# lab-emi/CleanUMamba

Measured on AMD Instinct MI355X. Metric: audio samples/sec/node (train step, E8, 10s@16kHz), higher is better.
Workload: dtype f16; 1 GPU; CleanUMamba-E8 (41.4M) full train step: fwd + L1 + multi-res STFT loss + bwd + grad all-reduce + clip + Adam; 10 s @ 16 kHz clips; global_batch=16, batch_per_gpu=16, clip_samples=160000, parallelism=dp1, weights=random init (reference init, seed 0)

## Files before the change

cleanumamba_amd/csrc/pack.hip:

```cpp
#include "common.h"

namespace cum {

template <typename TD>
struct Vec4;
template <>
struct Vec4<float> {
  typedef float4 type;
  static __device__ __forceinline__ type make(float a, float b, float c, float d) { return make_float4(a, b, c, d); }
};
template <>
struct Vec4<__bf16> {
  typedef __attribute__((ext_vector_type(4))) __bf16 type;
  static __device__ __forceinline__ type make(float a, float b, float c, float d) {
    type v = {(__bf16)a, (__bf16)b, (__bf16)c, (__bf16)d};
    return v;
  }
};

template <>
struct Vec4<f16> {
  typedef __attribute__((ext_vector_type(4))) _Float16 type;
  static __device__ __forceinline__ type make(float a, float b, float c, float d) {
    type v = {(f16)a, (f16)b, (f16)c, (f16)d};
    return v;
  }
};

template <typename TS, typename TD>
__global__ __launch_bounds__(256) void gather_kernel(const TS *__restrict__ src, const int32_t *__restrict__ idx,
                                                     TD *__restrict__ dst, int64_t n) {
  typedef typename Vec4<TD>::type V;
  const int64_t stride = (int64_t)gridDim.x * 256 * 8;
  for (int64_t i0 = ((int64_t)blockIdx.x * 256 + threadIdx.x) * 8; i0 < n; i0 += stride) {
    if (i0 + 7 < n) {
      const int4 j = *reinterpret_cast<const int4 *>(idx + i0), k = *reinterpret_cast<const int4 *>(idx + i0 + 4);
      const float v0 = j.x < 0 ? 0.f : (float)src[j.x], v1 = j.y < 0 ? 0.f : (float)src[j.y];
      const float v2 = j.z < 0 ? 0.f : (float)src[j.z], v3 = j.w < 0 ? 0.f : (float)src[j.w];
      const float v4 = k.x < 0 ? 0.f : (float)src[k.x], v5 = k.y < 0 ? 0.f : (float)src[k.y];
      const float v6 = k.z < 0 ? 0.f : (float)src[k.z], v7 = k.w < 0 ? 0.f : (float)src[k.w];
      *reinterpret_cast<V *>(dst + i0) = Vec4<TD>::make(v0, v1, v2, v3);
      *reinterpret_cast<V *>(dst + i0 + 4) = Vec4<TD>::make(v4, v5, v6, v7);
    } else {
      for (int64_t i = i0; i < n; ++i) {
        const int32_t jj = idx[i];
        dst[i] = (TD)(jj < 0 ? 0.f : (float)src[jj]);
      }
    }
  }
}

constexpr int PACK_PAD = -2147483647 - 1;
struct PackJob {
  int64_t dst_off;
  int32_t rows, cols;
  int32_t row_tab, col_tab;
  int32_t transpose;
  int32_t runs8;
};

template <typename TD>
__global__ __launch_bounds__(256) void pack2d_kernel(const float *__restrict__ src, const PackJob *__restrict__ jobs,
                                                    const int32_t *__restrict__ tiles, const int32_t *__restrict__ tables,
                                                    TD *__restrict__ dst) {
  typedef typename Vec4<TD>::type V;
  __shared__ __attribute__((aligned(16))) TD tile[64][72];
  const int tid = threadIdx.x;
  const PackJob j = jobs[tiles[3 * blockIdx.x]];
  const int r0 = tiles[3 * blockIdx.x + 1] * 64, c0 = tiles[3 * blockIdx.x + 2] * 64;
  const int32_t *rt = tables + j.row_tab, *ct = tables + j.col_tab;
  TD *out = dst + j.dst_off;
  if (j.transpose) {
    const int r = r0 + (tid & 63), cw = c0 + 16 * (tid >> 6);
    const int ro = r < j.rows ? rt[r] : PACK_PAD;
#pragma unroll
    for (int cc = 0; cc < 16; ++cc) {
      const int c = cw + cc;
      const int co = c < j.cols ? ct[c] : PACK_PAD;
      const float v = (ro == PACK_PAD || co == PACK_PAD) ? 0.f : src[(int64_t)ro + co];
      tile[tid & 63][16 * (tid >> 6) + cc] = (TD)v;
    }
    __syncthreads();
  }
  const int cg = 8 * (tid & 7);
#pragma unroll
  for (int h = 0; h < 2; ++h) {
    const int rl = (tid >> 3) + 32 * h, r = r0 + rl, c = c0 + cg;
    if (r >= j.rows || c >= j.cols) continue;
    if (j.transpose) {
      *reinterpret_cast<uint4 *>(out + (int64_t)r * j.cols + c) = *reinterpret_cast<const uint4 *>(&tile[rl][cg]);
      if constexpr (sizeof(TD) == 4)
        *reinterpret_cast<uint4 *>(out + (int64_t)r * j.cols + c + 4) = *reinterpret_cast<const uint4 *>(&tile[rl][cg + 4]);
    } else {
      const int ro = rt[r];
      float v[8];
      if (j.runs8) {
        const int co = ct[c];
        const bool pad = ro == PACK_PAD || co == PACK_PAD;
        const float *q = src + (pad ? 0 : (int64_t)ro + co);
        if (j.runs8 == 2) {
          const float4 a = pad ? make_float4(0.f, 0.f, 0.f, 0.f) : *reinterpret_cast<const float4 *>(q);
          const float4 b = pad ? make_float4(0.f, 0.f, 0.f, 0.f) : *reinterpret_cast<const float4 *>(q + 4);
          v[0] = a.x; v[1] = a.y; v[2] = a.z; v[3] = a.w; v[4] = b.x; v[5] = b.y; v[6] = b.z; v[7] = b.w;
        } else {
#pragma unroll
          for (int i = 0; i < 8; ++i) v[i] = pad ? 0.f : q[i];
        }
      } else {
#pragma unroll
        for (int i = 0; i < 8; ++i) {
          const int co = ct[c + i];
          v[i] = (ro == PACK_PAD || co == PACK_PAD) ? 0.f : src[(int64_t)ro + co];
        }
      }
      *reinterpret_cast<V *>(out + (int64_t)r * j.cols + c) = Vec4<TD>::make(v[0], v[1], v[2], v[3]);
      *reinterpret_cast<V *>(out + (int64_t)r * j.cols + c + 4) = Vec4<TD>::make(v[4], v[5], v[6], v[7]);
    }
  }
}

}

using namespace cum;

extern "C" int cum_pack2d(const float *src, const void *jobs, const int32_t *tiles, int32_t n_tiles, const int32_t *tables,
                          int32_t dst_dtype, void *dst, void *stream) {
  CUM_REQUIRE(dtype_ok(dst_dtype), "pack2d: dst dtype must be CUM_F32 / CUM_BF16 / CUM_F16");
  CUM_REQUIRE(n_tiles >= 0, "pack2d: negative tile count");
  if (n_tiles == 0) return CUM_OK;
  CUM_REQUIRE(src && jobs && tiles && tables && dst && ((uintptr_t)dst & 15) == 0 && ((uintptr_t)src & 15) == 0,
              "pack2d: null or misaligned pointer");
  hipStream_t st = (hipStream_t)stream;
  const PackJob *pj = static_cast<const PackJob *>(jobs);
  if (dst_dtype == CUM_F16)
    hipLaunchKernelGGL(pack2d_kernel<f16>, dim3(n_tiles), dim3(256), 0, st, src, pj, tiles, tables, (f16 *)dst);
  else if (dst_dtype == CUM_BF16)
    hipLaunchKernelGGL(pack2d_kernel<__bf16>, dim3(n_tiles), dim3(256), 0, st, src, pj, tiles, tables, (__bf16 *)dst);
  else
    hipLaunchKernelGGL(pack2d_kernel<float>, dim3(n_tiles), dim3(256), 0, st, src, pj, tiles, tables, (float *)dst);
  CUM_CHECK_LAUNCH();
  return CUM_OK;
}

extern "C" int cum_gather(int32_t src_dtype, const void *src, const int32_t *idx, int64_t n, int32_t dst_dtype,
                          void *dst, void *stream) {
  CUM_REQUIRE(dtype_ok(src_dtype) && dtype_ok(dst_dtype) && !(is16(src_dtype) && is16(dst_dtype) && src_dtype != dst_dtype),
              "gather: dtypes must be CUM_F32 / CUM_BF16 / CUM_F16 (no bf16 <-> f16 conversion)");
  CUM_REQUIRE(n >= 0, "gather: negative length");
  if (n == 0) return CUM_OK;
  CUM_REQUIRE(src && idx && dst && ((uintptr_t)idx & 15) == 0 && ((uintptr_t)dst & 15) == 0,
              "gather: null or misaligned pointer");
  const int64_t want = (n + 2047) / 2048;
  dim3 grid((unsigned)(want < 8192 ? want : 8192)), block(256);
  hipStream_t st = (hipStream_t)stream;
  if (src_dtype == CUM_F32 && dst_dtype == CUM_F16)
    hipLaunchKernelGGL((gather_kernel<float, f16>), grid, block, 0, st, (const float *)src, idx, (f16 *)dst, n);
  else if (src_dtype == CUM_F16 && dst_dtype == CUM_F32)
    hipLaunchKernelGGL((gather_kernel<f16, float>), grid, block, 0, st, (const f16 *)src, idx, (float *)dst, n);
  else if (src_dtype == CUM_F16)
    hipLaunchKernelGGL((gather_kernel<f16, f16>), grid, block, 0, st, (const f16 *)src, idx, (f16 *)dst, n);
  else if (src_dtype == CUM_F32 && dst_dtype == CUM_F32)
    hipLaunchKernelGGL((gather_kernel<float, float>), grid, block, 0, st, (const float *)src, idx, (float *)dst, n);
  else if (src_dtype == CUM_F32)
    hipLaunchKernelGGL((gather_kernel<float, __bf16>), grid, block, 0, st, (const float *)src, idx, (__bf16 *)dst, n);
  else if (dst_dtype == CUM_F32)
    hipLaunchKernelGGL((gather_kernel<__bf16, float>), grid, block, 0, st, (const __bf16 *)src, idx, (float *)dst, n);
  else
    hipLaunchKernelGGL((gather_kernel<__bf16, __bf16>), grid, block, 0, st, (const __bf16 *)src, idx, (__bf16 *)dst, n);
  CUM_CHECK_LAUNCH();
  return CUM_OK;
}
```

Measured before the change: 128.1 million audio samples/s.

## Make pack2d persistent with software-pipelined tile loads and double-buffered LDS

The pack kernel now launches a capped persistent grid sized to CU count times a fixed occupancy factor, and each workgroup walks a contiguous range of tiles. Table lookups and global loads for the next tile are issued while the current tile is being stored. LDS is double-buffered, and the non-transposed gather path now also goes through LDS. Branchy pad handling is replaced by redirecting padded reads to a zero buffer, with readlane broadcast of column indices. The aim is to hide gather latency and cut launch and tail overhead, at the cost of more registers and complexity in what is likely a small slice of the train step.

```diff
diff --git a/cleanumamba_amd/csrc/pack.hip b/cleanumamba_amd/csrc/pack.hip
--- a/cleanumamba_amd/csrc/pack.hip
+++ b/cleanumamba_amd/csrc/pack.hip
@@ -59,64 +59,169 @@
   int32_t runs8;
 };
 
+constexpr int PACK_WG_PER_CU = 8;
+
+struct PackTile {
+  int32_t job, tr, tc;
+};
+
+struct PackTab {
+  int32_t e0, e1, e2;
+};
+
+__device__ __forceinline__ bool pack_direct(const PackJob &j) { return !j.transpose && j.runs8; }
+
+__device__ __forceinline__ PackTile pack_tile(const int32_t *__restrict__ tiles, int t) {
+  PackTile p;
+  p.job = tiles[3 * t], p.tr = tiles[3 * t + 1], p.tc = tiles[3 * t + 2];
+  return p;
+}
+
+__device__ __forceinline__ PackTab pack_tab(const int32_t *__restrict__ tables, const PackJob &j, const PackTile &p,
+                                            int tid) {
+  const int32_t *rt = tables + j.row_tab, *ct = tables + j.col_tab;
+  PackTab t;
+  t.e2 = 0;
+  if (pack_direct(j)) {
+    const int r = 64 * p.tr + (tid >> 3), c = 64 * p.tc + 8 * (tid & 7);
+    t.e0 = rt[min(r, j.rows - 1)];
+    t.e1 = rt[min(r + 32, j.rows - 1)];
+    t.e2 = ct[min(c, j.cols - 8)];
+  } else if (j.transpose) {
+    t.e0 = rt[min(64 * p.tr + (tid & 63), j.rows - 1)];
+    t.e1 = ct[min(64 * p.tc + 16 * (tid >> 6) + (tid & 15), j.cols - 1)];
+  } else {
+    t.e0 = ct[min(64 * p.tc + (tid & 63), j.cols - 1)];
+    t.e1 = rt[min(64 * p.tr + 16 * (tid >> 6) + (tid & 15), j.rows - 1)];
+  }
+  return t;
+}
+
+__device__ __attribute__((aligned(16))) float pack_zeros[8];
+typedef float PackF4 __attribute__((ext_vector_type(4)));
+typedef const __attribute__((address_space(1))) float *PackSrc;
+typedef const __attribute__((address_space(1))) PackF4 *PackSrc4;
+
+__device__ __forceinline__ uintptr_t pack_addr(const float *src, int ro, int co, bool inside) {
+  const bool live = inside & (ro != PACK_PAD) & (co != PACK_PAD);
+  return live ? (uintptr_t)src + 4 * (uintptr_t)((int64_t)ro + co) : (uintptr_t)pack_zeros;
+}
+
+__device__ __forceinline__ void pack_load(const float *__restrict__ src, const PackJob &j, const PackTile &p, const PackTab &t,
+                                          int tid, float (&x)[16]) {
+  if (pack_direct(j)) {
+    const int r = 64 * p.tr + (tid >> 3);
+    const bool cin = 64 * p.tc + 8 * (tid & 7) < j.cols;
+#pragma unroll
+    for (int h = 0; h < 2; ++h) {
+      const uintptr_t q = pack_addr(src, h ? t.e1 : t.e0, t.e2, cin & (r + 32 * h < j.rows));
+      if (j.runs8 == 2) {
+        const PackF4 a = *(PackSrc4)q, b = *(PackSrc4)(q + 16);
+        x[8 * h + 0] = a.x, x[8 * h + 1] = a.y, x[8 * h + 2] = a.z, x[8 * h + 3] = a.w;
+        x[8 * h + 4] = b.x, x[8 * h + 5] = b.y, x[8 * h + 6] = b.z, x[8 * h + 7] = b.w;
+      } else {
+#pragma unroll
+        for (int i = 0; i < 8; ++i) x[8 * h + i] = *(PackSrc)(q + 4 * i);
+      }
+    }
+  } else {
+    const int own_n = j.transpose ? j.rows : j.cols, other_n = j.transpose ? j.cols : j.rows;
+    const bool own_in = 64 * (j.transpose ? p.tr : p.tc) + (tid & 63) < own_n;
+    const int first = 64 * (j.transpose ? p.tc : p.tr) + 16 * (tid >> 6);
+#pragma unroll
+    for (int k = 0; k < 16; ++k) {
+      const int e = __builtin_amdgcn_readlane(t.e1, k);
+      x[k] = *(PackSrc)pack_addr(src, t.e0, e, own_in & (first + k < other_n));
+    }
+  }
+}
+
+template <typename TD>
+__device__ __forceinline__ void pack_store8(TD *p, const float *v) {
+  typedef typename Vec4<TD>::type V;
+  if constexpr (sizeof(TD) == 4) {
+    *reinterpret_cast<V *>(p) = Vec4<TD>::make(v[0], v[1], v[2], v[3]);
+    *reinterpret_cast<V *>(p + 4) = Vec4<TD>::make(v[4], v[5], v[6], v[7]);
+  } else {
+    typedef TD V8 __attribute__((ext_vector_type(8)));
+    const V8 o = {(TD)v[0], (TD)v[1], (TD)v[2], (TD)v[3], (TD)v[4], (TD)v[5], (TD)v[6], (TD)v[7]};
+    *reinterpret_cast<V8 *>(p) = o;
+  }
+}
+
 template <typename TD>
 __global__ __launch_bounds__(256) void pack2d_kernel(const float *__restrict__ src, const PackJob *__restrict__ jobs,
-                                                    const int32_t *__restrict__ tiles, const int32_t *__restrict__ tables,
-                                                    TD *__restrict__ dst) {
-  typedef typename Vec4<TD>::type V;
-  __shared__ __attribute__((aligned(16))) TD tile[64][72];
+                                                    const int32_t *__restrict__ tiles, int32_t n_tiles,
+                                                    const int32_t *__restrict__ tables, TD *__restrict__ dst) {
+  __shared__ __attribute__((aligned(16))) TD tile[2][64][72];
   const int tid = threadIdx.x;
-  const PackJob j = jobs[tiles[3 * blockIdx.x]];
-  const int r0 = tiles[3 * blockIdx.x + 1] * 64, c0 = tiles[3 * blockIdx.x + 2] * 64;
-  const int32_t *rt = tables + j.row_tab, *ct = tables + j.col_tab;
-  TD *out = dst + j.dst_off;
-  if (j.transpose) {
-    const int r = r0 + (tid & 63), cw = c0 + 16 * (tid >> 6);
-    const int ro = r < j.rows ? rt[r] : PACK_PAD;
-#pragma unroll
-    for (int cc = 0; cc < 16; ++cc) {
-      const int c = cw + cc;
-      const int co = c < j.cols ? ct[c] : PACK_PAD;
-      const float v = (ro == PACK_PAD || co == PACK_PAD) ? 0.f : src[(int64_t)ro + co];
-      tile[tid & 63][16 * (tid >> 6) + cc] = (TD)v;
-    }
-    __syncthreads();
-  }
-  const int cg = 8 * (tid & 7);
-#pragma unroll
-  for (int h = 0; h < 2; ++h) {
-    const int rl = (tid >> 3) + 32 * h, r = r0 + rl, c = c0 + cg;
-    if (r >= j.rows || c >= j.cols) continue;
-    if (j.transpose) {
-      *reinterpret_cast<uint4 *>(out + (int64_t)r * j.cols + c) = *reinterpret_cast<const uint4 *>(&tile[rl][cg]);
-      if constexpr (sizeof(TD) == 4)
-        *reinterpret_cast<uint4 *>(out + (int64_t)r * j.cols + c + 4) = *reinterpret_cast<const uint4 *>(&tile[rl][cg + 4]);
+  const int t0 = (int)((int64_t)blockIdx.x * n_tiles / gridDim.x), t1 = (int)((int64_t)(blockIdx.x + 1) * n_tiles / gridDim.x);
+  if (t0 >= t1) return;
+  const int last = t1 - 1;
+  PackTile p0 = pack_tile(tiles, t0), p1 = pack_tile(tiles, min(t0 + 1, last)), p2 = pack_tile(tiles, min(t0 + 2, last)),
+           p3 = pack_tile(tiles, min(t0 + 3, last));
+  PackJob j0 = jobs[p0.job], j1 = jobs[p1.job], j2 = jobs[p2.job];
+  float xa[16], xb[16];
+#pragma unroll
+  for (int i = 0; i < 16; ++i) xa[i] = xb[i] = 0.f;
+  pack_load(src, j0, p0, pack_tab(tables, j0, p0, tid), tid, xa);
+  PackTab b1 = pack_tab(tables, j1, p1, tid);
+  int buf = 0;
+  auto step = [&](int t, float (&x)[16], float (&nx)[16]) {
+    const PackTab b2 = pack_tab(tables, j2, p2, tid);
+    if (t < last) pack_load(src, j1, p1, b1, tid, nx);
+    const PackJob j3 = jobs[p3.job];
+    const PackTile p4 = pack_tile(tiles, min(t + 4, last));
+    TD *out = dst + j0.dst_off;
+    const int r0 = 64 * p0.tr, c = 64 * p0.tc + 8 * (tid & 7);
+    if (!pack_direct(j0)) {
+      TD(*tl)[72] = tile[buf];
+      if (j0.transpose) {
+        pack_store8(&tl[tid & 63][16 * (tid >> 6)], x);
+        pack_store8(&tl[tid & 63][16 * (tid >> 6) + 8], x + 8);
+      } else {
+#pragma unroll
+        for (int k = 0; k < 16; ++k) tl[16 * (tid >> 6) + k][tid & 63] = (TD)x[k];
+      }
+      __syncthreads();
+#pragma unroll
+      for (int h = 0; h < 2; ++h) {
+        const int rl = (tid >> 3) + 32 * h, r = r0 + rl;
+        if (r >= j0.rows || c >= j0.cols) continue;
+        TD *o = out + (int64_t)r * j0.cols + c;
+        *reinterpret_cast<uint4 *>(o) = *reinterpret_cast<const uint4 *>(&tl[rl][8 * (tid & 7)]);
+        if constexpr (sizeof(TD) == 4)
+          *reinterpret_cast<uint4 *>(o + 4) = *reinterpret_cast<const uint4 *>(&tl[rl][8 * (tid & 7) + 4]);
+      }
+      buf ^= 1;
     } else {
-      const int ro = rt[r];
-      float v[8];
-      if (j.runs8) {
-        const int co = ct[c];
-        const bool pad = ro == PACK_PAD || co == PACK_PAD;
-        const float *q = src + (pad ? 0 : (int64_t)ro + co);
-        if (j.runs8 == 2) {
-          const float4 a = pad ? make_float4(0.f, 0.f, 0.f, 0.f) : *reinterpret_cast<const float4 *>(q);
-          const float4 b = pad ? make_float4(0.f, 0.f, 0.f, 0.f) : *reinterpret_cast<const float4 *>(q + 4);
-          v[0] = a.x; v[1] = a.y; v[2] = a.z; v[3] = a.w; v[4] = b.x; v[5] = b.y; v[6] = b.z; v[7] = b.w;
-        } else {
-#pragma unroll
-          for (int i = 0; i < 8; ++i) v[i] = pad ? 0.f : q[i];
-        }
-      } else {
-#pragma unroll
-        for (int i = 0; i < 8; ++i) {
-          const int co = ct[c + i];
-          v[i] = (ro == PACK_PAD || co == PACK_PAD) ? 0.f : src[(int64_t)ro + co];
-        }
-      }
-      *reinterpret_cast<V *>(out + (int64_t)r * j.cols + c) = Vec4<TD>::make(v[0], v[1], v[2], v[3]);
-      *reinterpret_cast<V *>(out + (int64_t)r * j.cols + c + 4) = Vec4<TD>::make(v[4], v[5], v[6], v[7]);
-    }
-  }
+#pragma unroll
+      for (int h = 0; h < 2; ++h) {
+        const int r = r0 + (tid >> 3) + 32 * h;
+        if (r >= j0.rows || c >= j0.cols) continue;
+        pack_store8(out + (int64_t)r * j0.cols + c, x + 8 * h);
+      }
+    }
+    p0 = p1, p1 = p2, p2 = p3, p3 = p4;
+    j0 = j1, j1 = j2, j2 = j3;
+    b1 = b2;
+  };
+  for (int t = t0; t < t1; t += 2) {
+    step(t, xa, xb);
+    if (t + 1 < t1) step(t + 1, xb, xa);
+  }
+}
+
+static int pack_cu_count() {
+  static int cus[64] = {};
+  int dev = 0;
+  if (hipGetDevice(&dev) != hipSuccess || dev < 0 || dev >= 64) return 0;
+  if (cus[dev] == 0) {
+    int n = 0;
+    if (hipDeviceGetAttribute(&n, hipDeviceAttributeMultiprocessorCount, dev) != hipSuccess || n <= 0) return 0;
+    cus[dev] = n;
+  }
+  return cus[dev];
 }
 
 }
@@ -130,14 +235,18 @@
   if (n_tiles == 0) return CUM_OK;
   CUM_REQUIRE(src && jobs && tiles && tables && dst && ((uintptr_t)dst & 15) == 0 && ((uintptr_t)src & 15) == 0,
               "pack2d: null or misaligned pointer");
+  const int cus = pack_cu_count();
+  CUM_REQUIRE(cus > 0, "pack2d: cannot read the device's CU count");
   hipStream_t st = (hipStream_t)stream;
   const PackJob *pj = static_cast<const PackJob *>(jobs);
+  const int64_t cap = (int64_t)cus * PACK_WG_PER_CU;
+  const dim3 grid((unsigned)(n_tiles < cap ? n_tiles : cap)), block(256);
   if (dst_dtype == CUM_F16)
-    hipLaunchKernelGGL(pack2d_kernel<f16>, dim3(n_tiles), dim3(256), 0, st, src, pj, tiles, tables, (f16 *)dst);
+    hipLaunchKernelGGL(pack2d_kernel<f16>, grid, block, 0, st, src, pj, tiles, n_tiles, tables, (f16 *)dst);
   else if (dst_dtype == CUM_BF16)
-    hipLaunchKernelGGL(pack2d_kernel<__bf16>, dim3(n_tiles), dim3(256), 0, st, src, pj, tiles, tables, (__bf16 *)dst);
+    hipLaunchKernelGGL(pack2d_kernel<__bf16>, grid, block, 0, st, src, pj, tiles, n_tiles, tables, (__bf16 *)dst);
   else
-    hipLaunchKernelGGL(pack2d_kernel<float>, dim3(n_tiles), dim3(256), 0, st, src, pj, tiles, tables, (float *)dst);
+    hipLaunchKernelGGL(pack2d_kernel<float>, grid, block, 0, st, src, pj, tiles, n_tiles, tables, (float *)dst);
   CUM_CHECK_LAUNCH();
   return CUM_OK;
 }
```

Measured after the change: 128.8 million audio samples/s (median of 6 runs). Within noise of the previous version (+0.5%).
